# facebookresearch/PointContrast

Hardware: AMD Instinct MI355X
Metric: scene-pairs/sec, ScanNet 2.5cm Res16UNet34C PointInfoNCE (higher is better)
Workload: dtype f32; 1 GPU; BASELINE configs[1]: Res16UNet34C, nce loss, voxel 0.025 m, 4 pairs/GPU, 87380+87371 active voxels per forward pair on rank 0, npos 4096, T 0.4, SGD(lr 0.1, mom 0.8, wd 1e-4); global_batch=4, parallelism=dp1, engine=native, pair_execution=one two-segment pass (BatchNorm statistics per cloud)

## Files before the change

pointcontrast_amd/build.py:

```python
import hashlib
import os
import subprocess
import sys
from concurrent.futures import ThreadPoolExecutor

HERE = os.path.dirname(os.path.abspath(__file__))
CSRC = os.path.join(HERE, "csrc")
BUILD = os.path.join(CSRC, "_build")
LIB = os.path.join(HERE, "libpcmi.so")
SOURCES = ["coords.hip", "spconv.hip", "spconv_x3.hip", "spconv_wgrad.hip", "spconv_wgrad_x3.hip", "spconv32r.hip", "norm.hip", "loss.hip", "nce_x3.hip", "engine.hip", "sortrows.hip", "widths.hip", "loader.hip", "pairs.hip", "pool.hip", "corpus.hip", "pointset.hip", "detect.hip", "evaldet.hip", "segeval.hip", "nearest.hip", "semseg_input.hip", "pair_input.hip", "detect_input.hip", "detect_features.hip", "votehead.hip", "rowspool.hip", "featmatch.hip"]
FLAGS = ["--offload-arch=gfx950", "-O3", "-std=c++17", "-fPIC", "-mcode-object-version=5", "-fno-slp-vectorize",
         "-Wall", "-Wno-unused-function"] + os.environ.get("PCMI_EXTRA_HIPCC_FLAGS", "").split()


def _hipcc():
  for c in (os.environ.get("HIPCC"), "/opt/rocm/bin/hipcc", "hipcc"):
    if c and (os.path.isabs(c) and os.path.exists(c) or not os.path.isabs(c)):
      return c
  raise RuntimeError("hipcc not found")


def _digest(paths):
  h = hashlib.sha256()
  for p in paths:
    with open(p, "rb") as f:
      h.update(f.read())
  h.update(" ".join(FLAGS).encode())
  return h.hexdigest()


def _headers():
  return [os.path.join(CSRC, "common.h"), os.path.join(CSRC, "internal.h"), os.path.join(CSRC, "spconv_args.h"), os.path.join(CSRC, "spconv_plan.h"),
          os.path.join(CSRC, "x3_split.h"), os.path.join(HERE, "..", "include", "pcmi.h")]


def sources_digest():
  return _digest([os.path.join(CSRC, s) for s in SOURCES] + _headers())


def build_variant(name, extra_flags, force=False, verbose=False):
  global BUILD, LIB, FLAGS
  saved = (BUILD, LIB, FLAGS)
  try:
    BUILD, LIB, FLAGS = os.path.join(CSRC, "_build_" + name), os.path.join(HERE, "libpcmi_%s.so" % name), FLAGS + list(extra_flags)
    return build_lib(force=force, verbose=verbose)
  finally:
    BUILD, LIB, FLAGS = saved


def build_lib(force=False, verbose=False):
  import fcntl
  try:
    os.makedirs(BUILD, exist_ok=True)
    lock = open(os.path.join(BUILD, ".lock"), "w")
  except PermissionError:
    return _build_locked(force, verbose)
  with lock:
    fcntl.flock(lock, fcntl.LOCK_EX)
    try:
      return _build_locked(force, verbose)
    finally:
      fcntl.flock(lock, fcntl.LOCK_UN)


def _build_locked(force, verbose):
  headers = _headers()
  hipcc = _hipcc()

  def compile_one(src):
    s = os.path.join(CSRC, src)
    o = os.path.join(BUILD, src.replace(".hip", ".o"))
    stamp = o + ".sha"
    dig = _digest([s] + headers)
    if not force and os.path.exists(o) and os.path.exists(stamp) and open(stamp).read() == dig:
      return o, False
    cmd = [hipcc] + FLAGS + ["-c", s, "-o", o]
    if verbose:
      print(" ".join(cmd), flush=True)
    r = subprocess.run(cmd, capture_output=True, text=True)
    if r.returncode != 0:
      raise RuntimeError("hipcc failed for %s:\n%s\n%s" % (src, r.stdout, r.stderr))
    with open(stamp, "w") as f:
      f.write(dig)
    return o, True

  with ThreadPoolExecutor(max_workers=min(8, len(SOURCES))) as ex:
    results = list(ex.map(compile_one, SOURCES))
  objs = [o for o, _ in results]
  if force or any(ch for _, ch in results) or not os.path.exists(LIB):
    tmp = LIB + ".tmp%d" % os.getpid()
    cmd = [hipcc, "--offload-arch=gfx950", "-shared", "-o", tmp] + objs
    if verbose:
      print(" ".join(cmd), flush=True)
    r = subprocess.run(cmd, capture_output=True, text=True)
    if r.returncode != 0:
      if os.path.exists(tmp):
        os.remove(tmp)
      raise RuntimeError("link failed:\n%s\n%s" % (r.stdout, r.stderr))
    os.replace(tmp, LIB)
  return LIB


if __name__ == "__main__":
  print(build_lib(force="--force" in sys.argv, verbose=True))
```

pointcontrast_amd/csrc/spconv.hip:

```cpp
#include <algorithm>
#include <cmath>
#include <cstdlib>

#include "common.h"
#include "internal.h"
#include "spconv_args.h"
#include "spconv_plan.h"

namespace pcmi {

typedef float f32x16 __attribute__((ext_vector_type(16)));
typedef float v4f __attribute__((ext_vector_type(4)));

constexpr int kKC = 32;


template <int NT, bool WT, int KC = kKC>
__device__ __forceinline__ void load_b_regs(v4f (&breg)[NT * KC / 32], const float* __restrict__ wb, int64_t w_sc,
                                            int64_t w_sn, int c0, int n0, int t) {
  constexpr int NS = 32 * NT;
#pragma unroll
  for (int i = 0; i < NT * KC / 32; ++i) {
    const int e = t + i * 256;
    if (!WT) {
      const int c = e / (NS / 4), n4 = e % (NS / 4);
      breg[i] = *reinterpret_cast<const v4f*>(wb + (int64_t)(c0 + c) * w_sc + n0 + n4 * 4);
    } else {
      const int n = e / (KC / 4), c4 = e % (KC / 4);
      breg[i] = *reinterpret_cast<const v4f*>(wb + (int64_t)(n0 + n) * w_sn + c0 + c4 * 4);
    }
  }
}

template <int NT, bool WT, int LDB, int KC = kKC>
__device__ __forceinline__ void store_b_regs(const v4f (&breg)[NT * KC / 32], float* __restrict__ sb, int t) {
  constexpr int NS = 32 * NT;
#pragma unroll
  for (int i = 0; i < NT * KC / 32; ++i) {
    const int e = t + i * 256;
    if (!WT) {
      const int c = e / (NS / 4), n4 = e % (NS / 4);
      *reinterpret_cast<v4f*>(sb + c * LDB + n4 * 4) = breg[i];
    } else {
      const int n = e / (KC / 4), c4 = e % (KC / 4);
      sb[(c4 * 4 + 0) * LDB + n] = breg[i].x;
      sb[(c4 * 4 + 1) * LDB + n] = breg[i].y;
      sb[(c4 * 4 + 2) * LDB + n] = breg[i].z;
      sb[(c4 * 4 + 3) * LDB + n] = breg[i].w;
    }
  }
}

template <int NT, int RW, bool WT, bool PAIR, int KC = kKC>
__global__ __launch_bounds__(256, KC > 32 ? 2 : 3) void spconv_mfma_kernel(ConvArgs a) {
  constexpr int TM = 32 * RW;
  constexpr int KG = 4 / RW;
  constexpr int BPG = KC / 8 / KG;
  constexpr int NS = 32 * NT;
  constexpr int LDB = WT ? NS + 1 : NS;
  constexpr int KSLOTS = PAIR ? 1 : PCMI_MAX_KERNEL_VOLUME;
  constexpr int STAGE_FLOATS = 2 * KC * LDB;
  constexpr int RED_FLOATS = (KG > 1) ? (KG - 1) * RW * 32 * NS : 0;
  constexpr int LDS_FLOATS = STAGE_FLOATS > RED_FLOATS ? STAGE_FLOATS : RED_FLOATS;

  __shared__ __attribute__((aligned(16))) float s_f[LDS_FLOATS];
  __shared__ int32_t s_idx[KSLOTS][TM];
  __shared__ int32_t s_orow[TM];
  __shared__ int32_t s_klist[KSLOTS];
  __shared__ int32_t s_nk;
  __shared__ int64_t s_tile[2];

  const int n0 = blockIdx.y * NS;
  const int t = threadIdx.x;
  const int lane = t & 63, wave = t >> 6;
  const int r = lane & 31, h = lane >> 5;
  const int rg = wave % RW, kg = wave / RW;
  int k_single = 0;
  if (PAIR) {
    if (t == 0) {
      int64_t tile = blockIdx.x, found_k = -1, p0 = 0;
      for (int k = 0; k < a.K; ++k) {
        const int64_t len = a.offs[k + 1] - a.offs[k];
        const int64_t nt = (len + TM - 1) / TM;
        if (tile < nt) {
          found_k = k;
          p0 = a.offs[k] + tile * TM;
          break;
// ... 193 lines not shown
  __shared__ int32_t s_orow[TM];
  __shared__ int2 s_kmeta[KSLOTS];
  __shared__ int32_t s_kabs[KSLOTS];
  __shared__ int32_t s_nk;
  __shared__ int64_t s_tile[2];

  const int n0 = blockIdx.y * NS;
  int sk_g = 0, sk_tile = 0, sk_u = 0, sk_u1 = 0;
  bool sk_first = true;
  if constexpr (SK) {
    const int G = (int)gridDim.x;
    sk_g = (int)(blockIdx.x & 7) * (G / 8) + (int)(blockIdx.x >> 3);
    const int U = a.sk_pref[a.sk_tiles] * (a.C / kKC);
    const int per = (U + G - 1) / G;
    sk_u = sk_g * per;
    sk_u1 = min(U, sk_u + per);
    if (sk_u >= sk_u1) return;
    if (threadIdx.x < 64) {
      int lo = 0, n = a.sk_tiles;
      while (n > 1) {
        const int stride = (n + 63) / 64;
        const int probe = lo + (int)threadIdx.x * stride;
        const bool le = probe < lo + n && a.sk_pref[probe] * (a.C / kKC) <= sk_u;
        const int cnt = __popcll(__ballot(le));
        const int nlo = lo + max(cnt - 1, 0) * stride;
        n = min(stride, lo + n - nlo);
        lo = nlo;
      }
      if (threadIdx.x == 0) s_tile[0] = lo;
    }
    __syncthreads();
    sk_tile = __builtin_amdgcn_readfirstlane((int)s_tile[0]);
  }
  const __amdgpu_buffer_rsrc_t xr = __builtin_amdgcn_make_buffer_rsrc(const_cast<float*>(a.x), 0, 0x7FFFFFFF, kRsrcFlags);
  const __amdgpu_buffer_rsrc_t wr = __builtin_amdgcn_make_buffer_rsrc(const_cast<float*>(a.w), 0, 0x7FFFFFFF, kRsrcFlags);
  const uint32_t ld_bytes = (uint32_t)(a.x_ld * 4);
  const uint32_t wk_bytes = (uint32_t)(a.w_kstride * 4);
  const int sk_total = SK ? sk_u1 - sk_u : 0;
  int sk_done = 0, prio_qtr = -1;
  for (;;) {
  bool sk_whole = true;
  int sk_next_u = 0, sk_c0 = 0, sk_steps = 0;
  int t = threadIdx.x;
  if constexpr (SK) asm volatile("" : "+v"(t));
  const int lane = t & 63, wave = t >> 6;
  const int i = lane & 15, kk = lane >> 4;
  if constexpr (SK) {
    const int64_t row0 = (int64_t)sk_tile * TM;
    const uint32_t tmask = a.sk_mask[sk_tile];
    const int nch_ = a.C / kKC;
    const int pref = a.sk_pref[sk_tile] * nch_, ns_t = __popc(tmask) * nch_;
    const int jb = sk_u - pref, je = min(sk_u1 - pref, ns_t);
    sk_whole = (jb == 0 && je == ns_t);
    sk_next_u = pref + je;
    const int o0 = jb / nch_, o1 = (je - 1) / nch_;
    sk_c0 = jb - o0 * nch_;
    sk_steps = je - jb;
    if (t < a.K && ((tmask >> t) & 1u)) {
      const int j = __popc(tmask & ((1u << t) - 1u));
      if (j >= o0 && j <= o1) {
        s_kabs[j - o0] = t;
        s_kmeta[j - o0] = make_int2(j - o0, (int)((uint32_t)a.wsel[t] * wk_bytes));
      }
    }
    if (t == 0) s_nk = sk_steps > 0 ? o1 - o0 + 1 : 0;
    if (t < TM) s_orow[t] = (row0 + t < a.n_rows) ? (a.perm ? a.perm[row0 + t] : (int32_t)(row0 + t)) : -1;
    __syncthreads();
    const int cnt = sk_steps > 0 ? o1 - o0 + 1 : 0;
    for (int p = t; p < cnt * TM; p += 256) {
      const int q = p / TM, rr = p - q * TM;
      const int64_t row = row0 + rr;
      const int32_t v = row < a.n_rows ? a.nbr[(int64_t)s_kabs[q] * a.n_rows + row] : -1;
      s_off[q][rr] = v >= 0 ? (uint32_t)v * ld_bytes : kAbsent;
    }
  } else {
    int64_t tile = blockIdx.x;
    if (a.xcd_tiles > 0) {
      tile = (int64_t)(blockIdx.x & 7) * a.xcd_tiles + (blockIdx.x >> 3);
      if (tile * TM >= a.n_rows) return;
    }
    const int64_t row0 = tile * TM;
    const int kbeg = (int)((int64_t)a.K * blockIdx.z / a.ksplit);
    const int kend = (int)((int64_t)a.K * (blockIdx.z + 1) / a.ksplit);
    if (t < TM) s_orow[t] = (row0 + t < a.n_rows) ? (a.perm ? a.perm[row0 + t] : (int32_t)(row0 + t)) : -1;
    for (int p = t; p < (kend - kbeg) * TM; p += 256) {
      const int q = p / TM, rr = p - q * TM;
      const int64_t row = row0 + rr;
      int32_t v = -1;
      if (row < a.n_rows) v = a.nbr ? a.nbr[(int64_t)(kbeg + q) * a.n_rows + row] : (int32_t)row;
      s_off[q][rr] = v >= 0 ? (uint32_t)v * ld_bytes : kAbsent;
    }
    __syncthreads();
    if (t < 64) {
      int nk = 0;
      for (int q = 0; q < kend - kbeg; ++q) {
        bool any = false;
        for (int rr = t; rr < TM; rr += 64) any |= (s_off[q][rr] != kAbsent);
        if (__any(any)) {
          if (t == 0) s_kmeta[nk] = make_int2(q, (int)((uint32_t)a.wsel[kbeg + q] * wk_bytes));
          ++nk;
        }
      }
      if (t == 0) s_nk = nk;
    }
  }
  __syncthreads();
  const int nk = s_nk;
  const int nch = a.C / kKC;
  const int nsteps = SK ? sk_steps : nk * nch;

  f32x4 acc[2][CTN];
#pragma unroll
  for (int g = 0; g < 2; ++g)
#pragma unroll
    for (int ct = 0; ct < CTN; ++ct) acc[g][ct] = (f32x4){0.f, 0.f, 0.f, 0.f};

  uint32_t bvo[NT];
#pragma unroll
  for (int q = 0; q < NT; ++q) {
    const int e = t + q * 256;
    if (!WT) {
      const int c = e / (NS / 4), n4 = e % (NS / 4);
      bvo[q] = (uint32_t)(((int64_t)c * a.w_sc + n0 + n4 * 4) * 4);
    } else {
      const int n = e / (kKC / 4), c4 = e % (kKC / 4);
      bvo[q] = (uint32_t)(((int64_t)(n0 + n) * a.w_sn + c4 * 4) * 4);
    }
  }
  const uint32_t b_chunk_bytes = (uint32_t)((WT ? (int64_t)kKC : (int64_t)kKC * a.w_sc) * 4);
  v4f breg[NT];
  auto store_b = [&](int buf) { store_b_regs<NT, WT, LDB>(breg, s_f + buf * (kKC * LDB), t); };
  v4f a0[2][2], a1[2][2];
  int va0 = 0, va1 = 0;
  int lj = 0, lc = sk_c0 - 1;
  int2 l_meta = make_int2(0, 0);
  uint32_t l_voff[2] = {kAbsent, kAbsent};
  const uint32_t off_lane = (uint32_t)(wave * 32 + i) * 4;
  auto stage_meta = [&]() {
    ++lc;
    if (lc == nch) {
      lc = 0;
      ++lj;
    }
    lc = __builtin_amdgcn_readfirstlane(lc);
    lj = __builtin_amdgcn_readfirstlane(lj);
    l_meta = s_kmeta[min(lj, KSLOTS - 1)];
  };
  auto stage_b = [&](bool live) {
    const int krow = __builtin_amdgcn_readfirstlane(l_meta.x) & 31;
    const uint32_t wofs = (uint32_t)__builtin_amdgcn_readfirstlane(l_meta.y);
    const char* row = reinterpret_cast<const char*>(&s_off[0][0]) + min(krow, KSLOTS - 1) * (TM * 4) + off_lane;
    l_voff[0] = *reinterpret_cast<const uint32_t*>(row);
    l_voff[1] = *reinterpret_cast<const uint32_t*>(row + 64);
    const uint32_t soff = (uint32_t)__builtin_amdgcn_readfirstlane((int)(wofs + (uint32_t)lc * b_chunk_bytes));
#pragma unroll
    for (int q = 0; q < NT; ++q)
      breg[q] = __builtin_bit_cast(v4f, __builtin_amdgcn_raw_buffer_load_b128(wr, live ? bvo[q] : kAbsent, live ? soff : 0u, 0));
  };
  auto stage_a = [&](v4f (&dst)[2][2], bool live) -> int {
    const uint32_t v0 = live ? l_voff[0] : kAbsent, v1 = live ? l_voff[1] : kAbsent;
    const int va = (__any(v0 != kAbsent) ? 1 : 0) | (__any(v1 != kAbsent) ? 2 : 0);
    const uint32_t soff = (uint32_t)__builtin_amdgcn_readfirstlane(lc * (kKC * 4));
    const uint32_t o0 = v0 + 16 * kk, o1 = v1 + 16 * kk;
    dst[0][0] = __builtin_bit_cast(v4f, __builtin_amdgcn_raw_buffer_load_b128(xr, o0, soff, 0));
    dst[1][0] = __builtin_bit_cast(v4f, __builtin_amdgcn_raw_buffer_load_b128(xr, o1, soff, 0));
    dst[0][1] = __builtin_bit_cast(v4f, __builtin_amdgcn_raw_buffer_load_b128(xr, o0 + 64, soff, 0));
    dst[1][1] = __builtin_bit_cast(v4f, __builtin_amdgcn_raw_buffer_load_b128(xr, o1 + 64, soff, 0));
    return va;
  };

  if (nsteps > 0) {
    stage_meta();
    stage_b(true);
// ... 272 lines not shown
  return PCMI_OK;
}

template <bool WT>
static int launch_deep(int NT, const ConvArgs& a, dim3 grid, hipStream_t st) {
  switch (NT) {
    case 1: spconv_mfma_kernel<1, 4, WT, false, 64><<<grid, 256, 0, st>>>(a); break;
    case 2: spconv_mfma_kernel<2, 4, WT, false, 64><<<grid, 256, 0, st>>>(a); break;
    default: set_error("spconv: bad NT %d", NT); return PCMI_ERR_INVALID;
  }
  PCMI_LAUNCH_CHECK();
  return PCMI_OK;
}

template <int RW, bool WT, bool PAIR>
static int launch_nt(int NT, const ConvArgs& a, dim3 grid, hipStream_t st) {
  switch (NT) {
    case 1: return launch_one<1, RW, WT, PAIR>(a, grid, st);
    case 2: return launch_one<2, RW, WT, PAIR>(a, grid, st);
    case 3: if constexpr (RW > 1) return launch_one<3, RW, WT, PAIR>(a, grid, st); else break;
    case 4: if constexpr (RW > 1) return launch_one<4, RW, WT, PAIR>(a, grid, st); else break;
  }
  set_error("spconv: bad NT %d", NT);
  return PCMI_ERR_INVALID;
}

template <bool WT, bool PAIR>
static int launch_rw(int RW, int NT, const ConvArgs& a, dim3 grid, hipStream_t st) {
  switch (RW) {
    case 4: return launch_nt<4, WT, PAIR>(NT, a, grid, st);
    case 2: return launch_nt<2, WT, PAIR>(NT, a, grid, st);
    case 1: return launch_nt<1, WT, PAIR>(NT, a, grid, st);
  }
  set_error("spconv: bad RW %d", RW);
  return PCMI_ERR_INVALID;
}

int x3_plan_nt(int64_t rows, int C, int N, int K) {
  if (C % 32 != 0 || N % 32 != 0 || C < 64 || N < 64 || K <= 1) return 0;
  const ConvPlan p = plan_conv(conv_env(), rows, 0, C, N, K, PCMI_CONV_FORM_TABLE);
  return p.kernel == PCMI_CONV_KERNEL_TABLE_X3 ? p.NT : 0;
}

static int run_gathered(const float* x, int64_t x_ld, int64_t x_rows, int C, const float* w, int cin, int cout,
                        bool w_transposed, int N, const pcmi_kmap_t* map, bool pair_mode,
                        bool swap_pairs, const int32_t* wsel, const float* bias, float* out,
                        int64_t out_ld, int64_t n_rows, int accumulate, void* ws, size_t ws_bytes,
                        hipStream_t st) {
  PCMI_REQUIRE(C % 32 == 0 && N % 32 == 0, PCMI_ERR_UNSUPPORTED,
               "spconv: channels (%d -> %d) must be multiples of 32 on the MFMA path", C, N);
  PCMI_REQUIRE(x_ld % 4 == 0 && out_ld >= N && out_ld % 4 == 0 && ((uintptr_t)x % 16 == 0) && ((uintptr_t)w % 16 == 0) &&
                   ((uintptr_t)out % 16 == 0),
               PCMI_ERR_INVALID, "spconv: operands must be 16-byte aligned with ld %% 4 == 0");
  if (n_rows == 0) return PCMI_OK;
  ConvArgs a = {};
  a.x = x;
  a.x_ld = x_ld;
  a.C = C;
  a.w = w;
  a.w_kstride = (int64_t)cin * cout;
  if (!w_transposed) {
    a.w_sc = cout;
    a.w_sn = 1;
  } else {
    a.w_sc = 1;
    a.w_sn = cout;
  }
  a.N = N;
  a.K = map ? map->K : 1;
  for (int k = 0; k < PCMI_MAX_KERNEL_VOLUME; ++k) a.wsel[k] = wsel ? wsel[k] : k;
  a.n_rows = n_rows;
  a.bias = bias;
  a.nbr = !map || pair_mode ? nullptr : map->nbr;
  a.ksplit = 1;
  a.accumulate = accumulate;
  a.out = out;
  a.out_ld = out_ld;
  int form = !map ? PCMI_CONV_FORM_NONE : pair_mode ? PCMI_CONV_FORM_PAIRS : PCMI_CONV_FORM_TABLE;
  if (form == PCMI_CONV_FORM_TABLE && map->perm && map->nbr_perm) {
    a.nbr = map->nbr_perm;
    a.perm = map->perm;
    if (map->tile_pref && map->n_tiles == ceil_div(n_rows, 128)) form = PCMI_CONV_FORM_TABLE_UNITS;
  }
  const ConvPlan p = plan_conv(conv_env(), n_rows, x_rows * x_ld * 4, C, N, a.K, form);
  PCMI_REQUIRE(p.ws_bytes == 0 || (ws && ws_bytes >= p.ws_bytes), PCMI_ERR_WORKSPACE, "spconv: workspace %zu < %zu bytes",
               ws_bytes, p.ws_bytes);
  const int terms = conv_terms();
  if (p.pack_bytes) {
    a.wpack = x3_find_prepacked(w, w_transposed, p.NT, terms);
    if (!a.wpack) {
      a.wpack = (char*)ws + p.pack_offset;
      const int rc_pack = x3_pack_weights(a, p.NT, const_cast<void*>(a.wpack), st, terms);
      if (rc_pack) return rc_pack;
    }
  }
  int rc;
  switch (p.kernel) {
    case PCMI_CONV_KERNEL_PAIR: {
      a.pair_src = swap_pairs ? map->pair_in : map->pair_out;
      a.pair_dst = swap_pairs ? map->pair_out : map->pair_in;
      a.offs = map->offs;
      const int TM = 32 * p.RW;
      int64_t tiles = 0;
      if (map->M >= 0)
        for (int k = 0; k < a.K; ++k) tiles += ceil_div(map->offs_host[k + 1] - map->offs_host[k], TM);
      else
        tiles = ceil_div(kmap_pairs_bound(*map), TM) + a.K;
      if (tiles == 0) return PCMI_OK;
      dim3 grid((unsigned)tiles, (unsigned)(N / (32 * p.NT)), 1);
      return w_transposed ? launch_rw<true, true>(p.RW, p.NT, a, grid, st) : launch_rw<false, true>(p.RW, p.NT, a, grid, st);
    }
    case PCMI_CONV_KERNEL_32R:
      return conv32r_launch(w_transposed, a, st);
    case PCMI_CONV_KERNEL_UNITS_16:
    case PCMI_CONV_KERNEL_UNITS_X3: {
      const bool x3 = p.kernel == PCMI_CONV_KERNEL_UNITS_X3;
      const int G = x3 ? x3_workgroups(p.NT, terms) : sk_workgroups(p.NT);
      a.sk_mask = map->tile_mask;
      a.sk_pref = map->tile_pref;
      a.sk_tiles = (int)map->n_tiles;
      a.sk_part = (float*)ws;
      dim3 grid((unsigned)G, (unsigned)(N / (32 * p.NT)), 1);
      if (x3)
        rc = x3_launch(p.NT, true, a, grid, st, terms);
      else
        rc = w_transposed ? launch16<true, true>(p.NT, a, grid, st) : launch16<false, true>(p.NT, a, grid, st);
      if (rc) return rc;
      const int sub = C / kKC;
      sk_fixup_kernel<<<dim3((unsigned)a.sk_tiles), 256, 0, st>>>(a.sk_part, a.sk_pref, a.sk_tiles, G, a.perm, n_rows, N, bias,
                                                                out, out_ld, accumulate, sub);
      PCMI_LAUNCH_CHECK();
      return PCMI_OK;
    }
  }
  if (p.ksplit > 1) {
    a.ksplit = p.ksplit;
    a.split_stride = n_rows * N;
    a.out = (float*)ws;
    a.out_ld = N;
    a.bias = nullptr;
    a.accumulate = 0;
  }
  int64_t tiles = ceil_div(n_rows, 32 * p.RW);
  if (tiles >= 64) {
    a.xcd_tiles = (int)ceil_div(tiles, 8);
    tiles = (int64_t)a.xcd_tiles * 8;
  }
  dim3 grid((unsigned)tiles, (unsigned)(N / (32 * p.NT)), (unsigned)p.ksplit);
  switch (p.kernel) {
    case PCMI_CONV_KERNEL_TABLE_X3: rc = x3_launch(p.NT, false, a, grid, st, terms); break;
    case PCMI_CONV_KERNEL_TABLE_16:
      rc = w_transposed ? launch16<true, false>(p.NT, a, grid, st) : launch16<false, false>(p.NT, a, grid, st);
      break;
    case PCMI_CONV_KERNEL_DEEP: rc = w_transposed ? launch_deep<true>(p.NT, a, grid, st) : launch_deep<false>(p.NT, a, grid, st); break;
    default: rc = w_transposed ? launch_rw<true, false>(p.RW, p.NT, a, grid, st) : launch_rw<false, false>(p.RW, p.NT, a, grid, st);
  }
  if (rc) return rc;
  if (p.ksplit > 1) {
    const int64_t n4 = n_rows * (N / 4);
    split_reduce_kernel<<<dim3((unsigned)ceil_div(n4, 256)), 256, 0, st>>>((const float*)ws, a.split_stride, p.ksplit,
                                                                         n_rows, N, bias, out, out_ld, accumulate);
    PCMI_LAUNCH_CHECK();
  }
  return PCMI_OK;
}

size_t spconv_fwd_bwd_workspace(int64_t n_in, int64_t n_out, int cin, int cout, int K) {
// ... 122 lines not shown
```

pointcontrast_amd/csrc/spconv_args.h:

```cpp
#pragma once
#include "common.h"

namespace pcmi {

struct ConvArgs {
  const float* x;
  int64_t x_ld;
  int C;
  const float* w;
  int64_t w_kstride;
  int64_t w_sc, w_sn;
  int N;
  const int32_t* nbr;
  const int32_t* perm;
  const int32_t* pair_src;
  const int32_t* pair_dst;
  const int64_t* offs;
  int K;
  int32_t wsel[PCMI_MAX_KERNEL_VOLUME];
  int64_t n_rows;
  float* out;
  int64_t out_ld;
  int64_t split_stride;
  int ksplit;
  const float* bias;
  int xcd_tiles;
  int accumulate;
  const uint32_t* sk_mask;
  const int32_t* sk_pref;
  int sk_tiles;
  float* sk_part;
  const void* wpack;
};

size_t x3_pack_bytes(int K, int C, int N);
int x3_pack_weights(const ConvArgs& a, int NT, void* out, hipStream_t st, int terms);
int x3_launch(int NT, bool sk, const ConvArgs& a, dim3 grid, hipStream_t st, int terms);
int x3_workgroups(int NT, int terms);
int x3_plan_nt(int64_t rows, int C, int N, int K);

bool conv32r_eligible(int64_t min_rows, int64_t rows, int64_t x_bytes, int C, int N, int K, bool table);
int conv32r_launch(bool w_transposed, const ConvArgs& a, hipStream_t st);

struct X3PackJob {
  const float* w;
  int64_t w_kstride, w_sc, w_sn;
  int K, C, N, NS;
  int terms;
  void* out;
  int64_t first_item;
};
int x3_pack_many(const X3PackJob* jobs_dev, int n_jobs, int64_t total_items, hipStream_t st, int64_t first_item = 0);
struct X3Prepacked {
  const float* w;
  int transposed;
  int NT;
  int terms;
  const void* pack;
};
void x3_set_prepacked(const X3Prepacked* table, int n);
const void* x3_find_prepacked(const float* w, bool transposed, int NT, int terms);

}
```

pointcontrast_amd/csrc/spconv_plan.h:

```cpp
#pragma once
#include <algorithm>
#include <cmath>
#include <cstdlib>

#include "internal.h"
#include "spconv_args.h"

namespace pcmi {

constexpr int kStreamKDefaultMinTiles = 256;

struct ConvEnv {
  int64_t sk_min_tiles, conv16_min_rows, conv32r_min_rows;
  bool x3_on;
};
static ConvEnv conv_env() {
  ConvEnv env;
  const char* e = getenv("PCMI_SPCONV_STREAMK");
  env.sk_min_tiles = e ? (int64_t)atoll(e) : (int64_t)kStreamKDefaultMinTiles;
  e = getenv("PCMI_CONV16");
  env.conv16_min_rows = e ? atoll(e) : 512;
  e = getenv("PCMI_CONV16_X3");
  env.x3_on = !e || atoi(e) != 0;
  e = getenv("PCMI_CONV32R");
  env.conv32r_min_rows = e ? (int64_t)atoll(e) : (int64_t)8192;
  return env;
}

static int sk_workgroups_max() { return 4 * num_cu() / 8 * 8; }
static bool sk_rows_eligible(const ConvEnv& env, int64_t rows, int K) {
  const int64_t mt = env.sk_min_tiles;
  return K > 1 && mt > 0 && rows >= 4096  && ceil_div(rows, 128) >= mt;
}
static size_t sk_partial_bytes(const ConvEnv& env, int64_t rows, int N, int K) {
  return sk_rows_eligible(env, rows, K) ? (size_t)sk_workgroups_max() * 2 * 128 * N * sizeof(float) : 0;
}

static bool conv16_enabled(const ConvEnv& env, int64_t n_rows, int64_t x_bytes) {
  const int64_t min_rows = env.conv16_min_rows;
  return min_rows > 0 && n_rows >= min_rows && x_bytes <= 0x7FFFFF00ll;
}

static bool conv16_x3(const ConvEnv& env, int NT, int C, int N) { return env.x3_on && NT >= 2 && NT <= 4 && C >= 64 && N >= 64; }

struct ConvPlan {
  int kernel;
  int RW, NT, ksplit;
  size_t split_bytes, sk_bytes, pack_offset, pack_bytes;
  size_t ws_bytes;
};
constexpr int kMaxKSplit = 27;

static ConvPlan plan_conv(const ConvEnv& env, int64_t rows, int64_t x_bytes, int C, int N, int K, int form) {
  ConvPlan p = {};
  const bool pair = form == PCMI_CONV_FORM_PAIRS, table = form == PCMI_CONV_FORM_TABLE || form == PCMI_CONV_FORM_TABLE_UNITS;
  p.ksplit = 1;
  if (conv32r_eligible(env.conv32r_min_rows, rows, x_bytes, C, N, K, table)) {
    p.kernel = PCMI_CONV_KERNEL_32R;
    return p;
  }
  const bool wide = C >= 64;
  const int nt_all = N / 32;
  p.NT = nt_all % 4 == 0 ? 4 : (nt_all % 3 == 0 ? 3 : (nt_all % 2 == 0 ? 2 : 1));
  p.RW = rows >= 96 ? 4 : (rows >= 48 ? 2 : 1);
  if (p.RW == 1 && p.NT > 2) p.NT = (nt_all % 2 == 0) ? 2 : 1;
  const int64_t min16 = env.conv16_min_rows;
  if (rows < 2048)
    p.NT = (wide && !pair && K > 1 && N >= 64 && nt_all % 2 == 0 && env.x3_on && min16 > 0 && rows >= min16 && p.RW == 4) ? 2 : 1;
  else if (rows < 8192 && p.NT > 2)
    p.NT = (nt_all % 2 == 0) ? 2 : 1;
  if (pair) {
    p.kernel = PCMI_CONV_KERNEL_PAIR;
    return p;
  }
  if (K > 1 && rows > 0) {
    const int64_t wgs = ceil_div(rows, 32 * p.RW) * (nt_all / p.NT);
    const int64_t target = (25 * (int64_t)num_cu()) / 10;
    if (wgs < target) p.ksplit = (int)std::min<int64_t>(std::min<int64_t>(K, kMaxKSplit), ceil_div(target, wgs));
    if (wide && p.RW == 4 && wgs < target && rows < 16384 && conv16_x3(env, p.NT, C, N) && min16 > 0 && rows >= min16) {
      const double slots = (double)x3_workgroups(p.NT, 3), nch = (double)(C / 32);
      const double traffic = (double)rows * N * 8.0 / 3.0e6 / 2.0;
      auto cost = [&](int ks) {
        const double w = (double)wgs * ks;
        const double rounds = std::ceil(w / slots);
        const double thin = std::max(1.0, 2.0 * num_cu() / std::min(w, slots));
        return rounds * ((double)ceil_div((int64_t)K, (int64_t)ks) * nch + 3.0) * thin + traffic * ks;
      };
      int best = p.ksplit;
      const int kmax = (int)std::min<int64_t>(K, kMaxKSplit);
      for (int ks = 1; ks <= kmax; ++ks)
        if (cost(ks) < cost(best) - 1e-9) best = ks;
      if (cost(best) < 0.9 * cost(p.ksplit)) p.ksplit = best;
    }
  }
  const bool c16 = p.RW == 4 && conv16_enabled(env, rows, x_bytes), x3 = conv16_x3(env, p.NT, C, N);
  if (form == PCMI_CONV_FORM_TABLE_UNITS && c16 && p.ksplit == 1 && sk_rows_eligible(env, rows, K) && C >= 64 && N >= 64) {
    p.kernel = x3 ? PCMI_CONV_KERNEL_UNITS_X3 : PCMI_CONV_KERNEL_UNITS_16;
    p.sk_bytes = sk_partial_bytes(env, rows, N, K);
    p.pack_offset = p.sk_bytes;
    p.pack_bytes = x3 ? x3_pack_bytes(K, C, N) : 0;
    p.ws_bytes = p.pack_offset + p.pack_bytes;
    return p;
  }
  p.split_bytes = p.ksplit > 1 ? (size_t)p.ksplit * rows * N * sizeof(float) : 0;
  p.ws_bytes = p.split_bytes;
  if (c16 && x3 && form != PCMI_CONV_FORM_NONE) {
    p.kernel = PCMI_CONV_KERNEL_TABLE_X3;
    p.pack_offset = align_up(p.split_bytes, 256);
// ... 14 lines not shown
```

pointcontrast_amd/csrc/spconv_x3.hip:

```cpp
#include <algorithm>
#include <cstdio>
#include <cstdlib>

#include "common.h"
#include "internal.h"
#include "spconv_args.h"
#include "x3_split.h"

namespace pcmi {

__host__ __device__ constexpr int x3_piece(int n, int kk) { return (n >> 4) * 64 + kk * 16 + (n & 15); }

__host__ __device__ constexpr int x3_channel(int kk, int e) { return 4 * kk + (e & 3) + 16 * (e >> 2); }

template <int TERMS>
__global__ __launch_bounds__(256) void x3_pack_kernel(const float* __restrict__ w, int64_t w_kstride, int64_t w_sc, int64_t w_sn,
                                                      int K, int C, int N, int NS, u32x4* __restrict__ out) {
  const int nch = C / kKC, nns = N / NS;
  const int64_t total = (int64_t)K * nch * nns * NS * 4;
  const int64_t idx = (int64_t)blockIdx.x * 256 + threadIdx.x;
  if (idx >= total) return;
  const int kk = (int)(idx & 3);
  int64_t r = idx >> 2;
  const int nl = (int)(r % NS);
  r /= NS;
  const int ns = (int)(r % nns);
  r /= nns;
  const int cc = (int)(r % nch);
  const int wk = (int)(r / nch);
  const float* wb = w + (int64_t)wk * w_kstride + (int64_t)(ns * NS + nl) * w_sn;
  v4f x0, x1;
#pragma unroll
  for (int e = 0; e < 4; ++e) {
    x0[e] = wb[(int64_t)(cc * kKC + x3_channel(kk, e)) * w_sc];
    x1[e] = wb[(int64_t)(cc * kKC + x3_channel(kk, e + 4)) * w_sc];
  }
  u32x4 h, m, l;
  split_terms<TERMS>(x0, x1, h, m, l);
  u32x4* blk = out + (((int64_t)wk * nch + cc) * nns + ns) * (TERMS * NS * 4);
  const int piece = x3_piece(nl, kk);
  blk[0 * NS * 4 + piece] = h;
  if constexpr (TERMS == 3) {
    blk[1 * NS * 4 + piece] = m;
    blk[2 * NS * 4 + piece] = l;
  }
}

__global__ __launch_bounds__(256) void x3_pack_many_kernel(const X3PackJob* __restrict__ jobs, int n_jobs, int64_t total,
                                                           int64_t item0) {
  const int64_t idx = item0 + (int64_t)blockIdx.x * 256 + threadIdx.x;
  if (idx >= total) return;
  int lo = 0, hi = n_jobs - 1;
  while (lo < hi) {
    const int mid = (lo + hi + 1) >> 1;
    if (jobs[mid].first_item <= idx) lo = mid; else hi = mid - 1;
  }
  const X3PackJob jb = jobs[lo];
  const int64_t loc = idx - jb.first_item;
  const int nch = jb.C / kKC, nns = jb.N / jb.NS;
  const int kk = (int)(loc & 3);
  int64_t r = loc >> 2;
  const int nl = (int)(r % jb.NS);
  r /= jb.NS;
  const int ns = (int)(r % nns);
  r /= nns;
  const int cc = (int)(r % nch);
  const int wk = (int)(r / nch);
  const float* wb = jb.w + (int64_t)wk * jb.w_kstride + (int64_t)(ns * jb.NS + nl) * jb.w_sn;
  v4f x0, x1;
#pragma unroll
  for (int e = 0; e < 4; ++e) {
    x0[e] = wb[(int64_t)(cc * kKC + x3_channel(kk, e)) * jb.w_sc];
    x1[e] = wb[(int64_t)(cc * kKC + x3_channel(kk, e + 4)) * jb.w_sc];
  }
  const int piece = x3_piece(nl, kk);
  if (jb.terms == 1) {
    u32x4 h;
    split1(x0, x1, h);
    reinterpret_cast<u32x4*>(jb.out)[(((int64_t)wk * nch + cc) * nns + ns) * (jb.NS * 4) + piece] = h;
    return;
  }
  u32x4 h, m, l;
  split3(x0, x1, h, m, l);
  u32x4* blk = reinterpret_cast<u32x4*>(jb.out) + (((int64_t)wk * nch + cc) * nns + ns) * (3 * jb.NS * 4);
  blk[0 * jb.NS * 4 + piece] = h;
  blk[1 * jb.NS * 4 + piece] = m;
  blk[2 * jb.NS * 4 + piece] = l;
// ... 26 lines not shown
  const uint32_t slice_bytes = (uint32_t)blockIdx.y * BLOCK_BYTES;
  int sk_g = 0, sk_tile = 0, sk_u = 0, sk_u1 = 0;
  bool sk_first = true;
  if constexpr (SK) {
    const int G = (int)gridDim.x;
    sk_g = (int)(blockIdx.x & 7) * (G / 8) + (int)(blockIdx.x >> 3);
    const int U = a.sk_pref[a.sk_tiles] * nch;
    const int per = (U + G - 1) / G;
    sk_u = sk_g * per;
    sk_u1 = min(U, sk_u + per);
    if (sk_u >= sk_u1) return;
    if (threadIdx.x < 64) {
      int lo = 0, n = a.sk_tiles;
      while (n > 1) {
        const int stride = (n + 63) / 64;
        const int probe = lo + (int)threadIdx.x * stride;
        const bool le = probe < lo + n && a.sk_pref[probe] * nch <= sk_u;
        const int cnt = __popcll(__ballot(le));
        const int nlo = lo + max(cnt - 1, 0) * stride;
        n = min(stride, lo + n - nlo);
        lo = nlo;
      }
      if (threadIdx.x == 0) s_tile[0] = lo;
    }
    __syncthreads();
    sk_tile = __builtin_amdgcn_readfirstlane((int)s_tile[0]);
  }
  const __amdgpu_buffer_rsrc_t xr = __builtin_amdgcn_make_buffer_rsrc(const_cast<float*>(a.x), 0, 0x7FFFFFFF, kRsrcFlags);
  const __amdgpu_buffer_rsrc_t wr = __builtin_amdgcn_make_buffer_rsrc(const_cast<void*>(a.wpack), 0, 0x7FFFFFFF, kRsrcFlags);
  const uint32_t ld_bytes = (uint32_t)(a.x_ld * 4);
  const int sk_total = SK ? sk_u1 - sk_u : 0;
  int sk_done = 0, prio_qtr = -1;
  for (;;) {
  bool sk_whole = true;
  int sk_next_u = 0, sk_c0 = 0, sk_steps = 0;
  int t = threadIdx.x;
  if constexpr (SK) asm volatile("" : "+v"(t));
  const int lane = t & 63, wave = t >> 6;
  const int i = lane & 15, kk = lane >> 4;
  if constexpr (SK) {
    const int64_t row0 = (int64_t)sk_tile * TM;
    const uint32_t tmask = a.sk_mask[sk_tile];
    const int pref = a.sk_pref[sk_tile] * nch, ns_t = __popc(tmask) * nch;
    const int jb = sk_u - pref, je = min(sk_u1 - pref, ns_t);
    sk_whole = (jb == 0 && je == ns_t);
    sk_next_u = pref + je;
    const int o0 = jb / nch, o1 = (je - 1) / nch;
    sk_c0 = jb - o0 * nch;
    sk_steps = je - jb;
    if (t < a.K && ((tmask >> t) & 1u)) {
      const int j = __popc(tmask & ((1u << t) - 1u));
      if (j >= o0 && j <= o1) {
        s_kabs[j - o0] = t;
        s_kmeta[j - o0] = make_int2(j - o0, (int)((uint32_t)a.wsel[t] * wk_bytes + slice_bytes));
      }
    }
    if (t == 0) s_nk = sk_steps > 0 ? o1 - o0 + 1 : 0;
    if (t < TM) s_orow[t] = (row0 + t < a.n_rows) ? (a.perm ? a.perm[row0 + t] : (int32_t)(row0 + t)) : -1;
    __syncthreads();
    const int cnt = sk_steps > 0 ? o1 - o0 + 1 : 0;
    {
      const int rr = t & (TM - 1);
      const int64_t row = row0 + rr;
      const bool row_ok = row < a.n_rows;
      const int64_t row_c = row_ok ? row : a.n_rows - 1;
      for (int q0 = t >> 7; q0 < cnt; q0 += 8) {
        int32_t v[4];
#pragma unroll
        for (int u = 0; u < 4; ++u) v[u] = a.nbr[(int64_t)s_kabs[min(q0 + 2 * u, cnt - 1)] * a.n_rows + row_c];
#pragma unroll
        for (int u = 0; u < 4; ++u)
          if (q0 + 2 * u < cnt) s_off[q0 + 2 * u][rr] = (row_ok && v[u] >= 0) ? (uint32_t)v[u] * ld_bytes : kAbsent;
      }
    }
  } else {
    int64_t tile = blockIdx.x;
    if (a.xcd_tiles > 0) {
      tile = (int64_t)(blockIdx.x & 7) * a.xcd_tiles + (blockIdx.x >> 3);
      if (tile * TM >= a.n_rows) return;
    }
    const int64_t row0 = tile * TM;
    const int kbeg = (int)((int64_t)a.K * blockIdx.z / a.ksplit);
    const int kend = (int)((int64_t)a.K * (blockIdx.z + 1) / a.ksplit);
    if (t < TM) s_orow[t] = (row0 + t < a.n_rows) ? (a.perm ? a.perm[row0 + t] : (int32_t)(row0 + t)) : -1;
    for (int p = t; p < (kend - kbeg) * TM; p += 256) {
      const int q = p / TM, rr = p - q * TM;
      const int64_t row = row0 + rr;
      int32_t v = -1;
      if (row < a.n_rows) v = a.nbr ? a.nbr[(int64_t)(kbeg + q) * a.n_rows + row] : (int32_t)row;
      s_off[q][rr] = v >= 0 ? (uint32_t)v * ld_bytes : kAbsent;
    }
    __syncthreads();
    if (t < 64) {
      int nk = 0;
      for (int q = 0; q < kend - kbeg; ++q) {
        bool any = false;
        for (int rr = t; rr < TM; rr += 64) any |= (s_off[q][rr] != kAbsent);
        if (__any(any)) {
          if (t == 0) s_kmeta[nk] = make_int2(q, (int)((uint32_t)a.wsel[kbeg + q] * wk_bytes + slice_bytes));
          ++nk;
        }
      }
      if (t == 0) s_nk = nk;
    }
  }
  __syncthreads();
  const int nk = s_nk;
  const int nsteps = SK ? sk_steps : nk * nch;

  f32x4 acc[2][CTN];
#pragma unroll
  for (int g = 0; g < 2; ++g)
#pragma unroll
    for (int ct = 0; ct < CTN; ++ct) acc[g][ct] = (f32x4){0.f, 0.f, 0.f, 0.f};

  constexpr int BRR = DMA ? 1 : BR;
  uint32_t bvo[BRR];
#pragma unroll
  for (int q = 0; q < BRR; ++q) bvo[q] = (t + q * 256 < PIECES) ? (uint32_t)(t + q * 256) * 16u : kAbsent;
  u32x4 breg[BRR];
  auto store_b = [&](int buf) {
    if constexpr (!DMA) {
#pragma unroll
      for (int q = 0; q < BR; ++q)
        if ((q + 1) * 256 <= PIECES || t + q * 256 < PIECES) s_b[buf][t + q * 256] = breg[q];
    }
  };
  constexpr int WPIECES = PIECES / 64, WR = (WPIECES + 3) / 4;
  const int wave_u = __builtin_amdgcn_readfirstlane(wave);
  auto dma_b = [&](int buf, uint32_t soff) {
    if constexpr (DMA) {
#pragma unroll
      for (int r = 0; r < WR; ++r) {
        const int wp = wave_u + 4 * r;
        if (wp < WPIECES)
          __builtin_amdgcn_raw_ptr_buffer_load_lds(wr, (__attribute__((address_space(3))) void*)&s_b[buf][wp * 64], 16,
                                                   (uint32_t)lane * 16u,
                                                   (uint32_t)__builtin_amdgcn_readfirstlane((int)(soff + (uint32_t)wp * 1024u)), 0, 0);
      }
    }
  };
  v4f a0[2][2], a1[2][2];
  int va0 = 0, va1 = 0;
  int lj = 0, lc = sk_c0 - 1;
  int2 l_meta = make_int2(0, 0);
  uint32_t l_voff[2] = {kAbsent, kAbsent};
  const uint32_t off_lane = (uint32_t)(wave * 32 + i) * 4;
  auto stage_meta = [&]() {
    ++lc;
    if (lc == nch) {
      lc = 0;
      ++lj;
    }
    lc = __builtin_amdgcn_readfirstlane(lc);
    lj = __builtin_amdgcn_readfirstlane(lj);
    l_meta = s_kmeta[min(lj, KSLOTS - 1)];
  };
  auto stage_b = [&](bool live, int nbuf) {
    const int krow = __builtin_amdgcn_readfirstlane(l_meta.x) & 31;
    const uint32_t wofs = (uint32_t)__builtin_amdgcn_readfirstlane(l_meta.y);
    const char* row = reinterpret_cast<const char*>(&s_off[0][0]) + min(krow, KSLOTS - 1) * (TM * 4) + off_lane;
    l_voff[0] = *reinterpret_cast<const uint32_t*>(row);
    l_voff[1] = *reinterpret_cast<const uint32_t*>(row + 64);
    const uint32_t soff = (uint32_t)__builtin_amdgcn_readfirstlane((int)(wofs + (uint32_t)lc * chunk_bytes));
    if constexpr (DMA) {
      if (live) dma_b(nbuf, soff);
    } else {
#pragma unroll
      for (int q = 0; q < BR; ++q)
        breg[q] = __builtin_bit_cast(u32x4, __builtin_amdgcn_raw_buffer_load_b128(wr, live ? bvo[q] : kAbsent, live ? soff : 0u, 0));
    }
  };
  auto stage_a = [&](v4f (&dst)[2][2], bool live) -> int {
// ... 195 lines not shown
```

Baseline: 294.9 scene-pairs/sec.

## Regroup rows within conv16 tiles by neighbour-presence mask to skip empty offsets

```diff
diff --git a/pointcontrast_amd/build.py b/pointcontrast_amd/build.py
--- a/pointcontrast_amd/build.py
+++ b/pointcontrast_amd/build.py
@@ -31,6 +31,7 @@
 
 def _headers():
   return [os.path.join(CSRC, "common.h"), os.path.join(CSRC, "internal.h"), os.path.join(CSRC, "spconv_args.h"), os.path.join(CSRC, "spconv_plan.h"),
+          os.path.join(CSRC, "conv16_regroup.h"),
           os.path.join(CSRC, "x3_split.h"), os.path.join(HERE, "..", "include", "pcmi.h")]
 
 
diff --git a/pointcontrast_amd/csrc/conv16_regroup.h b/pointcontrast_amd/csrc/conv16_regroup.h
--- /dev/null
+++ b/pointcontrast_amd/csrc/conv16_regroup.h
@@ -0,0 +1,63 @@
+#pragma once
+#include "spconv_args.h"
+
+namespace pcmi {
+
+constexpr int kRegroupScratchBytes = 128 * 4 + 128 * 4;
+constexpr int kRegroupMaxOffsets = 32 - 7;
+
+__device__ __forceinline__ bool conv16_regroup_applies(const ConvArgs& a, int cnt) {
+  return a.regroup && a.nbr && !a.perm && a.K > 8 && cnt <= kRegroupMaxOffsets;
+}
+
+__host__ __device__ constexpr int conv16_regroup_slot(int rank) { return ((rank >> 4) & 3) * 32 + (rank >> 6) * 16 + (rank & 15); }
+
+template <int TM, int KSLOTS>
+__device__ __forceinline__ void conv16_load_regrouped(const ConvArgs& a, int64_t row0, int kbeg, int cnt, uint32_t ld_bytes,
+                                                      uint32_t (&s_off)[KSLOTS][TM], int32_t (&s_orow)[TM], void* scratch, int t) {
+  static_assert(TM == 128, "7 bits of row");
+  constexpr int QMAX = KSLOTS < kRegroupMaxOffsets ? KSLOTS : kRegroupMaxOffsets;
+  constexpr uint32_t kAbsent = 0x80000000u;
+  uint32_t* s_key = reinterpret_cast<uint32_t*>(scratch);
+  int32_t* s_above = reinterpret_cast<int32_t*>(s_key + TM);
+  const int rr = t & (TM - 1);
+  const int half = __builtin_amdgcn_readfirstlane(t >> 7);
+  int32_t v[QMAX];
+  const int64_t row = row0 + rr;
+  const bool row_ok = row < a.n_rows;
+  if (half == 0) {
+    const int64_t row_c = row_ok ? row : a.n_rows - 1;
+#pragma unroll
+    for (int q = 0; q < QMAX; ++q) {
+      v[q] = -1;
+      if (q < cnt) v[q] = a.nbr[(int64_t)(kbeg + q) * a.n_rows + row_c];
+    }
+    uint32_t m = 0;
+#pragma unroll
+    for (int q = 0; q < QMAX; ++q) {
+      if (!row_ok) v[q] = -1;
+      m |= (v[q] >= 0 ? 1u : 0u) << q;
+    }
+    s_key[rr] = (m << 7) | (uint32_t)(TM - 1 - rr);
+  }
+  __syncthreads();
+  const uint32_t mine = s_key[rr];
+  const uint4* keys = reinterpret_cast<const uint4*>(s_key) + half * (TM / 8);
+  int above = 0;
+#pragma unroll
+  for (int u = 0; u < TM / 8; ++u) {
+    const uint4 k = keys[u];
+    above += (k.x > mine ? 1 : 0) + (k.y > mine ? 1 : 0) + (k.z > mine ? 1 : 0) + (k.w > mine ? 1 : 0);
+  }
+  if (half != 0) s_above[rr] = above;
+  __syncthreads();
+  if (half == 0) {
+    const int slot = conv16_regroup_slot(above + s_above[rr]);
+    s_orow[slot] = row_ok ? (int32_t)row : -1;
+#pragma unroll
+    for (int q = 0; q < QMAX; ++q)
+      if (q < cnt) s_off[q][slot] = v[q] >= 0 ? (uint32_t)v[q] * ld_bytes : kAbsent;
+  }
+}
+
+}
diff --git a/pointcontrast_amd/csrc/spconv.hip b/pointcontrast_amd/csrc/spconv.hip
--- a/pointcontrast_amd/csrc/spconv.hip
+++ b/pointcontrast_amd/csrc/spconv.hip
@@ -3,6 +3,7 @@
 #include <cstdlib>
 
 #include "common.h"
+#include "conv16_regroup.h"
 #include "internal.h"
 #include "spconv_args.h"
 #include "spconv_plan.h"
@@ -362,13 +363,18 @@
     const int64_t row0 = tile * TM;
     const int kbeg = (int)((int64_t)a.K * blockIdx.z / a.ksplit);
     const int kend = (int)((int64_t)a.K * (blockIdx.z + 1) / a.ksplit);
-    if (t < TM) s_orow[t] = (row0 + t < a.n_rows) ? (a.perm ? a.perm[row0 + t] : (int32_t)(row0 + t)) : -1;
-    for (int p = t; p < (kend - kbeg) * TM; p += 256) {
-      const int q = p / TM, rr = p - q * TM;
-      const int64_t row = row0 + rr;
-      int32_t v = -1;
-      if (row < a.n_rows) v = a.nbr ? a.nbr[(int64_t)(kbeg + q) * a.n_rows + row] : (int32_t)row;
-      s_off[q][rr] = v >= 0 ? (uint32_t)v * ld_bytes : kAbsent;
+    if (conv16_regroup_applies(a, kend - kbeg)) {
+      static_assert(sizeof(s_f) >= kRegroupScratchBytes, "the weight staging area is lent to the regrouping");
+      conv16_load_regrouped<TM, KSLOTS>(a, row0, kbeg, kend - kbeg, ld_bytes, s_off, s_orow, s_f, t);
+    } else {
+      if (t < TM) s_orow[t] = (row0 + t < a.n_rows) ? (a.perm ? a.perm[row0 + t] : (int32_t)(row0 + t)) : -1;
+      for (int p = t; p < (kend - kbeg) * TM; p += 256) {
+        const int q = p / TM, rr = p - q * TM;
+        const int64_t row = row0 + rr;
+        int32_t v = -1;
+        if (row < a.n_rows) v = a.nbr ? a.nbr[(int64_t)(kbeg + q) * a.n_rows + row] : (int32_t)row;
+        s_off[q][rr] = v >= 0 ? (uint32_t)v * ld_bytes : kAbsent;
+      }
     }
     __syncthreads();
     if (t < 64) {
@@ -807,7 +813,9 @@
     a.perm = map->perm;
     if (map->tile_pref && map->n_tiles == ceil_div(n_rows, 128)) form = PCMI_CONV_FORM_TABLE_UNITS;
   }
-  const ConvPlan p = plan_conv(conv_env(), n_rows, x_rows * x_ld * 4, C, N, a.K, form);
+  const ConvEnv env = conv_env();
+  a.regroup = env.regroup16 ? 1 : 0;
+  const ConvPlan p = plan_conv(env, n_rows, x_rows * x_ld * 4, C, N, a.K, form);
   PCMI_REQUIRE(p.ws_bytes == 0 || (ws && ws_bytes >= p.ws_bytes), PCMI_ERR_WORKSPACE, "spconv: workspace %zu < %zu bytes",
                ws_bytes, p.ws_bytes);
   const int terms = conv_terms();
diff --git a/pointcontrast_amd/csrc/spconv_args.h b/pointcontrast_amd/csrc/spconv_args.h
--- a/pointcontrast_amd/csrc/spconv_args.h
+++ b/pointcontrast_amd/csrc/spconv_args.h
@@ -26,6 +26,7 @@
   const float* bias;
   int xcd_tiles;
   int accumulate;
+  int regroup;
   const uint32_t* sk_mask;
   const int32_t* sk_pref;
   int sk_tiles;
diff --git a/pointcontrast_amd/csrc/spconv_plan.h b/pointcontrast_amd/csrc/spconv_plan.h
--- a/pointcontrast_amd/csrc/spconv_plan.h
+++ b/pointcontrast_amd/csrc/spconv_plan.h
@@ -12,7 +12,7 @@
 
 struct ConvEnv {
   int64_t sk_min_tiles, conv16_min_rows, conv32r_min_rows;
-  bool x3_on;
+  bool x3_on, regroup16;
 };
 static ConvEnv conv_env() {
   ConvEnv env;
@@ -24,6 +24,8 @@
   env.x3_on = !e || atoi(e) != 0;
   e = getenv("PCMI_CONV32R");
   env.conv32r_min_rows = e ? (int64_t)atoll(e) : (int64_t)8192;
+  e = getenv("PCMI_CONV16_REGROUP");
+  env.regroup16 = !e || atoi(e) != 0;
   return env;
 }
 
diff --git a/pointcontrast_amd/csrc/spconv_x3.hip b/pointcontrast_amd/csrc/spconv_x3.hip
--- a/pointcontrast_amd/csrc/spconv_x3.hip
+++ b/pointcontrast_amd/csrc/spconv_x3.hip
@@ -3,6 +3,7 @@
 #include <cstdlib>
 
 #include "common.h"
+#include "conv16_regroup.h"
 #include "internal.h"
 #include "spconv_args.h"
 #include "x3_split.h"
@@ -195,13 +196,18 @@
     const int64_t row0 = tile * TM;
     const int kbeg = (int)((int64_t)a.K * blockIdx.z / a.ksplit);
     const int kend = (int)((int64_t)a.K * (blockIdx.z + 1) / a.ksplit);
-    if (t < TM) s_orow[t] = (row0 + t < a.n_rows) ? (a.perm ? a.perm[row0 + t] : (int32_t)(row0 + t)) : -1;
-    for (int p = t; p < (kend - kbeg) * TM; p += 256) {
-      const int q = p / TM, rr = p - q * TM;
-      const int64_t row = row0 + rr;
-      int32_t v = -1;
-      if (row < a.n_rows) v = a.nbr ? a.nbr[(int64_t)(kbeg + q) * a.n_rows + row] : (int32_t)row;
-      s_off[q][rr] = v >= 0 ? (uint32_t)v * ld_bytes : kAbsent;
+    if (conv16_regroup_applies(a, kend - kbeg)) {
+      static_assert(sizeof(s_b) >= kRegroupScratchBytes, "the weight staging area is lent to the regrouping");
+      conv16_load_regrouped<TM, KSLOTS>(a, row0, kbeg, kend - kbeg, ld_bytes, s_off, s_orow, &s_b[0][0], t);
+    } else {
+      if (t < TM) s_orow[t] = (row0 + t < a.n_rows) ? (a.perm ? a.perm[row0 + t] : (int32_t)(row0 + t)) : -1;
+      for (int p = t; p < (kend - kbeg) * TM; p += 256) {
+        const int q = p / TM, rr = p - q * TM;
+        const int64_t row = row0 + rr;
+        int32_t v = -1;
+        if (row < a.n_rows) v = a.nbr ? a.nbr[(int64_t)(kbeg + q) * a.n_rows + row] : (int32_t)row;
+        s_off[q][rr] = v >= 0 ? (uint32_t)v * ld_bytes : kAbsent;
+      }
     }
     __syncthreads();
     if (t < 64) {
```

Measured after the change: 295.6 scene-pairs/sec (median of 2 runs). Within noise of the previous version (+0.2%).
